# RustAudio/lewton

Hardware: NVIDIA H100
Metric: Msamples/s IMDCT+window+OLA, 2048-pt long blocks (higher is better)
Workload: dtype f32

## Files before the change

### lewton_b200/csrc/host_objects.cuh

```cuda
#pragma once

struct DevBuf {
    void *p = nullptr;
    size_t cap = 0;
};

struct Staging {
    void *h = nullptr;
    size_t cap = 0;
    cudaEvent_t ev = nullptr;
    bool pending = false;
};

struct ArenaSet {
    DevBuf coeffs, dense, pcm, kinds, ys, vqoff, vqrec;
    cudaEvent_t done = nullptr;
};
constexpr int kHostSets = 2;

struct CachedTables {
    DevTables dt;
    std::vector<float> a, b, c, w;
    std::vector<uint32_t> br;
    std::vector<void *> allocs;
};

struct lwb_ctx {
    int device = 0;
    int sm_count = 0;
    cudaStream_t stream = nullptr;
    cudaStream_t copy_in = nullptr, copy_out = nullptr;
    cudaEvent_t ev_in[64] = {}, ev_done[65] = {};
    DevBuf runs_buf[2];
    cudaEvent_t ev_desc[2] = {}, ev_kdone[2] = {};
    int runs_par = 0;
    uint32_t ticket_next = 0;
    uint64_t epoch = 0;
    uint64_t state_gen = 1;
    std::string err;
    uint64_t launches = 0;
    uint64_t kernel_launches[LWB_KERNEL_COUNT] = {};
    std::vector<PcmSpan> pcm_spans;
    std::vector<PcmCopy> pcm_copies;
    std::deque<CachedTables> tables;
    DevBuf spec, segtab, magic, x, desc, chains, ticket, cdesc, cbytes;
    DevBuf floor0;
    ArenaSet host_sets[kHostSets];
    int host_next = 0;
    ArenaSet ordered;
    Staging stage[3];
    int stage_next = 0;
    std::vector<void *> stage_old;
    uint64_t tickets_issued = 0, tickets_done = 0;
    std::deque<cudaEvent_t> ticket_events;
    std::vector<cudaEvent_t> spare_events;
    bool pinned_only = false;
    void *h_desc = nullptr;
    size_t h_desc_cap = 0;
    size_t x_cap_elems = (size_t)64 << 20;
};

struct lwb_setup {
    lwb_ctx *ctx = nullptr;
    DevSetup host;
    DevSetup *d_setup = nullptr;
    std::vector<void *> allocs;
    uint8_t channels = 0, bs0 = 0, bs1 = 0;
    uint32_t n_modes = 0;
    uint32_t n_mappings = 0;
    std::vector<DevMapping> mappings;
    std::vector<uint8_t> floor_types;
    std::vector<DevFloor0> floor0;
    mutable bool streams_opened = false;
    bool floor0_described(uint32_t fi) const { return fi < floor0.size() && floor0[fi].order != 0; }
};

struct RowCopy { const float *src; float *dst; uint32_t n4, pad; };
struct ChainShape { unsigned warps; size_t smem; int n1max, wpc, np; };

struct Step {
    int kernel;
    const void *desc;
    size_t n;
    const float *pack;
};

struct StepArgs {
    void *pcm = nullptr;
    int out_format = LWB_OUT_F32_PLANAR;
    const float *w_short = nullptr;
    int ls = 0;
    int mid_kb = 0;
    ChainShape chain = {};
    const uint8_t *bytes = nullptr;
    bool residue = false;
    const float *coeffs = nullptr, *dense = nullptr;
    const uint8_t *kinds = nullptr;
    const uint32_t *ys = nullptr;
    const float *zero = nullptr;
};
// ... 10 lines not shown
    bool dense = false;
    bool floor0 = false;
};

struct lwb_plan {
    lwb_ctx *ctx = nullptr;
    lwb_chain *chains = nullptr;
    size_t n_chains = 0;
    lwb_batch_io io;
    bool captured = false;
    uint64_t gen = 0;
    FrontStages front;
    DevBuf pro, mix;
    StepArgs args;
    std::vector<Step> steps;
};

struct lwb_stream {
    lwb_ctx *ctx = nullptr;
    const lwb_setup *setup = nullptr;
    float *d_state = nullptr;
    bool has = false;
    uint32_t plen = 0;
    uint64_t busy_epoch = 0;
};

static void capture(lwb_plan *plan, uint64_t gen, const FrontStages &front, const StepArgs &args, std::vector<Step> steps)
{
    plan->captured = true;
    plan->gen = gen;
    plan->front = front;
    for (size_t i = 0; i < plan->n_chains && front.n; i++)
        if (!plan->chains[i].stream->setup->floor0.empty()) plan->front.floor0 = true;
    plan->args = args;
    plan->steps = std::move(steps);
}


static inline void set_stream_state(lwb_stream *s, bool has, uint32_t plen)
{
    if (s->has != has || s->plen != plen) {
        s->has = has;
        s->plen = plen;
        s->ctx->state_gen++;
    }
}

static int fail(lwb_ctx *ctx, int code, const char *what, cudaError_t e = cudaSuccess)
{
    if (ctx) {
        ctx->err = what;
        if (e != cudaSuccess) {
            ctx->err += ": ";
            ctx->err += cudaGetErrorString(e);
        }
    }
    return code;
}

static inline void count_launch(lwb_ctx *ctx, int kernel_id)
{
    ctx->launches++;
    ctx->kernel_launches[kernel_id]++;
}

#define CU(ctx, call)                                                        \
// ... 211 lines not shown
```

### lewton_b200/csrc/kernel_long.cuh

```cuda
#pragma once
#include <stdint.h>

#if defined(__CUDACC__)
#include <cuda_runtime.h>
#define LWB_HD __host__ __device__ __forceinline__
#else
#define LWB_HD inline
#endif

namespace lwb {

constexpr int kLongBs = 11;
constexpr int kLongN = 2048;
constexpr int kLongN2 = 1024;

struct alignas(16) LongRun {
    const float *in;
    void *out;
    float *state;
    uint32_t in_stride;
    uint32_t n_packets;
    uint8_t has_prev;
    uint8_t write_state;
    uint8_t dummy;
    uint8_t first_short;
    uint8_t last_short;
    uint8_t pad[3];
    float *state_out;
};
static_assert(sizeof(LongRun) == 48, "LongRun is copied by TMA in 16-byte units");

struct V { float x, y; };

#if defined(__CUDA_ARCH__)
__device__ __forceinline__ V vadd(V a, V b) { return V{__fadd_rn(a.x, b.x), __fadd_rn(a.y, b.y)}; }
__device__ __forceinline__ V vsub(V a, V b) { return V{__fsub_rn(a.x, b.x), __fsub_rn(a.y, b.y)}; }
__device__ __forceinline__ V vmul(V a, V b) { return V{__fmul_rn(a.x, b.x), __fmul_rn(a.y, b.y)}; }
__device__ __forceinline__ V vadd_p(V a, V b) { return V{__fadd_rn(a.x, b.x), __fadd_rn(a.y, b.y)}; }
__device__ __forceinline__ V vsub_p(V a, V b) { return V{__fsub_rn(a.x, b.x), __fsub_rn(a.y, b.y)}; }
__device__ __forceinline__ V vnsub_p(V a, V b) { return V{__fsub_rn(-a.x, b.x), __fsub_rn(-a.y, b.y)}; }
#else
inline V vadd(V a, V b) { return V{a.x + b.x, a.y + b.y}; }
inline V vsub(V a, V b) { return V{a.x - b.x, a.y - b.y}; }
inline V vmul(V a, V b) { return V{a.x * b.x, a.y * b.y}; }
inline V vadd_p(V a, V b) { return vadd(a, b); }
inline V vsub_p(V a, V b) { return vsub(a, b); }
inline V vnsub_p(V a, V b) { return V{-a.x - b.x, -a.y - b.y}; }
#endif

enum {
// ... 389 lines not shown
    }
};

__device__ __forceinline__ uint32_t laneA(int lane, int half) { return 4u * (uint32_t)swz(elemA(lane, 0, half)); }
__device__ __forceinline__ uint32_t laneB(int lane) { return 4u * (uint32_t)swz(elemB(lane, 0, 0)); }
__device__ __forceinline__ uint32_t laneC(int lane, int half) { return 4u * (uint32_t)swz(elemC(lane, 0, half)); }
#define LWB_KA(j) (4u * (uint32_t)swz(64 * (j)))
#define LWB_KB(j, h) (4u * (uint32_t)swz(((h) << 6) | ((j) << 3)))
#define LWB_KC(j) (4u * (uint32_t)swz(j))

struct RunCur {
    const float *in;
    void *out;
    float *state;
    uint32_t in_stride;
    uint32_t flags;
};
__device__ __forceinline__ RunCur run_cur(const LongRun &r)
{
    return RunCur{r.in, r.out, r.state, r.in_stride,
                  (uint32_t)(r.has_prev ? 1u : 0u) | (r.write_state ? 2u : 0u) | (r.dummy ? 4u : 0u) |
                      (r.first_short ? 8u : 0u) | (r.last_short ? 16u : 0u)};
}
struct RunCurS : RunCur { float *state_out; };
__device__ __forceinline__ RunCurS run_cur_s(const LongRun &r)
{
    RunCurS c;
    static_cast<RunCur &>(c) = run_cur(r);
    c.flags |= r.first_short == 2 ? 32u : 0u;
    c.state_out = r.state_out ? r.state_out : r.state;
    return c;
}

__device__ __forceinline__ int16_t d_sample_i16(float v)
{
    short r;
    asm("cvt.rzi.s16.f32 %0, %1;" : "=h"(r) : "f"(__fmul_rn(v, 32768.0f)));
    return (int16_t)r;
}
__device__ __forceinline__ void st_pcm(float *p, float v) { __stcs(p, v); }
__device__ __forceinline__ void st_pcm(int16_t *p, float v) { __stcs(reinterpret_cast<short *>(p), (short)d_sample_i16(v)); }

template <int NB, bool FIRST, typename OutT, typename RC = RunCur>
__device__ __forceinline__ void out_stage(const TwMix &tw, int lane, const V O[NB][8], const V E[NB][8], V pe[NB][8],
                                          const RC cur[NB], OutT *out[NB], const float *s_state)
{
// ... 142 lines not shown
    uint32_t desc_parity = 0;
    RunCur cur[NB];
    uint32_t npk;

    auto issue_stage = [&](uint32_t stage, const LongRun *r, uint32_t pkt) {
        const uint32_t bar = bars_s + 8 * stage;
        mbar_expect_tx(bar, kLongStageBytes);
#pragma unroll
        for (int b = 0; b < NB; b++)
            tma_load_1d(tiles_s + stage * kLongStageBytes + b * kLongTileBytes,
                        r[b].in + (size_t)pkt * r[b].in_stride, kLongTileBytes, bar);
    };
    auto issue_stage_cur = [&](uint32_t stage, uint32_t pkt) {
        const uint32_t bar = bars_s + 8 * stage;
        mbar_expect_tx(bar, kLongStageBytes);
#pragma unroll
        for (int b = 0; b < NB; b++)
            tma_load_1d(tiles_s + stage * kLongStageBytes + b * kLongTileBytes,
                        cur[b].in + (size_t)pkt * cur[b].in_stride, kLongTileBytes, bar);
    };
    auto issue_state = [&](const float *const st[NB], const uint32_t has[NB]) {
        uint32_t bytes = 0;
#pragma unroll
        for (int b = 0; b < NB; b++) bytes += has[b] ? kLongTileBytes : 0;
        mbar_expect_tx(bar_state, bytes);
#pragma unroll
        for (int b = 0; b < NB; b++)
            if (has[b]) tma_load_1d(state_s + b * kLongTileBytes, st[b], kLongTileBytes, bar_state);
    };

    {
        uint32_t idx = 0;
        if (lane == 0) idx = atomicAdd(ticket, 1u);
        idx = __shfl_sync(0xffffffffu, idx, 0);
        if (idx >= n_groups) return;
#pragma unroll
        for (int b = 0; b < NB; b++) cur[b] = run_cur(runs[idx * NB + b]);
        npk = runs[idx * NB].n_packets;
        if (lane == 0) {
            fence_proxy_async();
            const float *st[NB];
            uint32_t has[NB];
#pragma unroll
            for (int b = 0; b < NB; b++) { st[b] = cur[b].state; has[b] = cur[b].flags & 1u; }
            issue_state(st, has);
            for (; lc < (uint32_t)kLongRing && lc < npk; lc++) issue_stage_cur(lc, lc);
            nx_idx = atomicAdd(ticket, 1u);
        }
    }

    for (;;) {
        V pe[NB][8];
#pragma unroll
        for (int b = 0; b < NB; b++)
#pragma unroll
            for (int j = 0; j < 8; j++) pe[b][j] = V{0.f, 0.f};
        OutT *out[NB];
#pragma unroll
        for (int b = 0; b < NB; b++) out[b] = static_cast<OutT *>(cur[b].out);

        for (uint32_t p = 0; p < npk; p++) {
            const uint32_t stage_s = tiles_s + slot_i * kLongStageBytes;
            mbar_wait(bars_s + 8 * slot_i, (phase_bits >> slot_i) & 1u);
            phase_bits ^= 1u << slot_i;

            V O[NB][8], E[NB][8];
            {
// ... 67 lines not shown
                        lc++;
                    } else {
                        if (nx_stage == 1) {
                            mbar_wait(bar_desc, desc_parity);
                            desc_parity ^= 1u;
                            nx_stage = 2;
                            nx_npk = s_next[0].n_packets;
                            nx_lc = 0;
                        }
                        if (nx_stage == 2 && nx_lc < nx_npk) {
                            fence_proxy_async();
                            issue_stage(tgt, s_next, nx_lc);
                            nx_lc++;
                        }
                    }
                }
            }
            phase_c_fft<NB>(tw, O, E);
            if (p > 0) {
                out_stage<NB, false, OutT>(tw, lane, O, E, pe, cur, out, s_state);
            } else {
                mbar_wait(bar_state, (phase_bits >> 30) & 1u);
                phase_bits ^= 1u << 30;
                if (NB == 1 && (cur[0].flags & 8u))
                    out_first_short<NB, OutT>(tw, lane, O, E, pe, cur, out, s_state, w_short, ls);
                else
                    out_stage<NB, true, OutT>(tw, lane, O, E, pe, cur, out, s_state);
                __syncwarp();
            }
#pragma unroll
            for (int b = 0; b < NB; b++)
                if (p > 0 || (cur[b].flags & 1u)) out[b] += (p == 0 && (cur[b].flags & 8u)) ? kLongN2 - ls : kLongN2;
            if (lane == 0 && nx_stage == 2 && !nx_state_issued) {
                const float *st[NB];
                uint32_t has[NB];
#pragma unroll
                for (int b = 0; b < NB; b++) { st[b] = s_next[b].state; has[b] = s_next[b].has_prev; }
                fence_proxy_async();
                issue_state(st, has);
                nx_state_issued = 1;
            }
            slot_i = (slot_i + 1 == (uint32_t)kLongRing) ? 0 : slot_i + 1;
        }
#pragma unroll
        for (int b = 0; b < NB; b++) {
            if ((cur[b].flags & 16u)) {
                const bool emitted = (npk > 1 || (cur[b].flags & 1u)) && !(cur[b].flags & 4u);
                const bool keep = (cur[b].flags & 6u) == 2u;
#pragma unroll
                for (int j = 0; j < 8; j++) {
                    const int r64 = 64 * rev3(j);
#pragma unroll
                    for (int h = 0; h < 2; h++) {
                        const float v = ((j & 1) != 0) == (h == 0) ? pe[b][j].x : pe[b][j].y;
                        const int m = r64 + (h ? 63 - lane : lane);
                        if (m < ls) {
                            if (emitted) st_pcm(out[b] + m, v);
                        } else if (keep && m < kLongN2 - ls) {
                            cur[b].state[m - ls] = v;
                            cur[b].state[kLongN2 - 1 - ls - m] = v;
                        }
                    }
                }
            } else if ((cur[b].flags & 6u) == 2u) {
                float *s_lo = cur[b].state + lane, *s_hi = cur[b].state + 63 - lane;
#pragma unroll
                for (int j = 0; j < 8; j++) {
                    const int r64 = 64 * rev3(j);
                    const float vx = (j & 1) ? pe[b][j].x : pe[b][j].y, vy = (j & 1) ? pe[b][j].y : pe[b][j].x;
                    s_lo[r64] = vx; s_hi[r64] = vy;
                    s_hi[960 - r64] = vx; s_lo[960 - r64] = vy;
                }
            }
        }
        uint32_t st_ = 0, nlc = 0;
        if (lane == 0) {
            if (nx_stage == 0) {
                if (nx_idx < n_groups) {
                    fence_proxy_async();
                    mbar_expect_tx(bar_desc, NB * (uint32_t)sizeof(LongRun));
                    tma_load_1d(next_s, runs + (size_t)nx_idx * NB, NB * (uint32_t)sizeof(LongRun), bar_desc);
                    nx_stage = 1;
                } else {
                    nx_stage = 3;
                }
            }
            if (nx_stage == 1) {
                mbar_wait(bar_desc, desc_parity);
                desc_parity ^= 1u;
                nx_stage = 2;
                nx_npk = s_next[0].n_packets;
                nx_lc = 0;
            }
            if (nx_stage == 2 && !nx_state_issued) {
                const float *st[NB];
                uint32_t has[NB];
#pragma unroll
                for (int b = 0; b < NB; b++) { st[b] = s_next[b].state; has[b] = s_next[b].has_prev; }
                fence_proxy_async();
                issue_state(st, has);
            }
            st_ = nx_stage;
            nlc = nx_lc;
        }
        st_ = __shfl_sync(0xffffffffu, st_, 0);
        nlc = __shfl_sync(0xffffffffu, nlc, 0);
        if (st_ != 2) break;
        __syncwarp();
#pragma unroll
        for (int b = 0; b < NB; b++) cur[b] = run_cur(s_next[b]);
        npk = s_next[0].n_packets;
        __syncwarp();
        lc = nlc;
        nx_stage = 0; nx_lc = 0; nx_npk = 0; nx_state_issued = 0;
        if (lane == 0) {
            fence_proxy_async();
            for (uint32_t k = lc; k < (uint32_t)kLongRing && k < npk; k++) {
                issue_stage_cur((slot_i + k) % kLongRing, k);
                lc = k + 1;
            }
            nx_idx = atomicAdd(ticket, 1u);
        }
    }
}

constexpr int kLongLs256 = (kLongN - 256) / 4;
constexpr int kLongFetch = 3;
constexpr int kLongDescSlots = kLongFetch + kLongRing + 3;
constexpr int kLongSlopeMax = 512;
constexpr size_t kLongSmemBytesS = 2048 + (size_t)kLongWarps * (kLongRing + 1) * kLongTileBytes + (size_t)kLongPackFloats * 4 +
                                   kLongWarps * (kLongRing + 2) * 8 + (size_t)kLongWarps * kLongDescSlots * sizeof(LongRun) +
                                   kLongSlopeMax * sizeof(float) + 64;

// ... 218 lines not shown
```

### lewton_b200/csrc/lwb_api.cu

```cuda
#include <cuda_runtime.h>
#include <sched.h>
#include <sys/syscall.h>
#include <unistd.h>

#include <algorithm>
#include <cctype>
#include <cstdio>
#include <cstdlib>
#include <cstring>
#include <deque>
#include <new>
#include <string>
#include <vector>

#include "kernel_long.cuh"
#include "kernel_short.cuh"
#include "kernel_mid.cuh"
#include "kernels_generic.cuh"
#include "kernel_chain.cuh"
#include "kernel_prologue.cuh"
#include "kernel_floor0.cuh"
#include "lwb_common.h"
#include "pcm_copy_plan.h"
#include "../../include/lewton_frontend.h"
// ... 55 lines not shown
    short_kernel_configure();
    mid_kernel_configure();
    prologue_kernel_configure();
    *out = ctx;
    return LWB_OK;
}

static cudaError_t sync_all_streams(lwb_ctx *ctx)
{
    cudaError_t e = cudaStreamSynchronize(ctx->stream);
    for (cudaStream_t s : {ctx->copy_in, ctx->copy_out}) {
        const cudaError_t e2 = s ? cudaStreamSynchronize(s) : cudaSuccess;
        if (e == cudaSuccess) e = e2;
    }
    return e;
}

extern "C" void lwb_ctx_destroy(lwb_ctx *ctx)
{
    if (!ctx) return;
    cudaSetDevice(ctx->device);
    sync_all_streams(ctx);
    for (DevBuf *b : {&ctx->spec, &ctx->segtab, &ctx->magic, &ctx->x, &ctx->desc, &ctx->chains, &ctx->ticket, &ctx->runs_buf[0],
                      &ctx->runs_buf[1], &ctx->cdesc, &ctx->cbytes, &ctx->floor0})
        if (b->p) cudaFree(b->p);
    auto free_set = [](ArenaSet &s) {
        for (DevBuf *b : {&s.coeffs, &s.dense, &s.pcm, &s.kinds, &s.ys, &s.vqoff, &s.vqrec})
            if (b->p) cudaFree(b->p);
        if (s.done) cudaEventDestroy(s.done);
    };
    for (ArenaSet &s : ctx->host_sets) free_set(s);
    free_set(ctx->ordered);
    for (cudaEvent_t e : ctx->ticket_events) cudaEventDestroy(e);
    for (cudaEvent_t e : ctx->spare_events) cudaEventDestroy(e);
    for (CachedTables &ct : ctx->tables)
        for (void *p : ct.allocs) cudaFree(p);
    if (ctx->h_desc) cudaFreeHost(ctx->h_desc);
    for (void *h : ctx->stage_old) cudaFreeHost(h);
    for (Staging &st : ctx->stage) {
        if (st.h) cudaFreeHost(st.h);
        if (st.ev) cudaEventDestroy(st.ev);
    }
    for (cudaEvent_t e : ctx->ev_in) if (e) cudaEventDestroy(e);
    for (cudaEvent_t e : ctx->ev_done) if (e) cudaEventDestroy(e);
    for (int k = 0; k < 2; k++) {
        if (ctx->ev_desc[k]) cudaEventDestroy(ctx->ev_desc[k]);
        if (ctx->ev_kdone[k]) cudaEventDestroy(ctx->ev_kdone[k]);
// ... 386 lines not shown
    if (!s) return;
    cudaSetDevice(s->ctx->device);
    sync_all_streams(s->ctx);
    cudaFree(s->d_state);
    delete s;
}

extern "C" int lwb_stream_reset(lwb_stream *s)
{
    if (!s) return LWB_ERR_INVALID;
    set_stream_state(s, false, 0);
    return LWB_OK;
}
extern "C" int lwb_stream_is_empty(const lwb_stream *s) { return (!s || !s->has) ? 1 : 0; }
extern "C" uint32_t lwb_stream_state_len(const lwb_stream *s) { return (s && s->has) ? s->plen : 0; }

extern "C" int lwb_stream_clone(const lwb_stream *s, lwb_stream **out)
{
    if (!s || !out) return LWB_ERR_INVALID;
    int rc = lwb_stream_open(s->ctx, s->setup, out);
    if (rc) return rc;
    (*out)->has = s->has;
    (*out)->plen = s->plen;
    lwb_ctx *ctx = s->ctx;
    CU(ctx, cudaMemcpyAsync((*out)->d_state, s->d_state,
                            s->setup->channels * state_stride(s->setup) * sizeof(float),
                            cudaMemcpyDeviceToDevice, ctx->stream));
    return LWB_OK;
}

extern "C" int lwb_stream_export_state(lwb_stream *s, float *out)
{
    if (!s || !out) return LWB_ERR_INVALID;
    if (!s->has) return LWB_OK;
    lwb_ctx *ctx = s->ctx;
    CU(ctx, cudaSetDevice(ctx->device));
    CU(ctx, cudaMemcpy2DAsync(out, s->plen * sizeof(float), s->d_state, state_stride(s->setup) * sizeof(float),
                              s->plen * sizeof(float), s->setup->channels, cudaMemcpyDeviceToHost, ctx->stream));
    CU(ctx, cudaStreamSynchronize(ctx->stream));
    return LWB_OK;
}

extern "C" int lwb_stream_import_state(lwb_stream *s, const float *data, uint32_t len)
{
    if (!s || (!data && len)) return LWB_ERR_INVALID;
    if (len > state_stride(s->setup)) return LWB_ERR_BUFFER;
    lwb_ctx *ctx = s->ctx;
    CU(ctx, cudaSetDevice(ctx->device));
    if (len) {
        CU(ctx, cudaMemcpy2DAsync(s->d_state, state_stride(s->setup) * sizeof(float), data, len * sizeof(float),
                                  len * sizeof(float), s->setup->channels, cudaMemcpyHostToDevice, ctx->stream));
        CU(ctx, cudaStreamSynchronize(ctx->stream));
    }
    s->ctx->state_gen++;
    s->has = true;
    s->plen = len;
    return LWB_OK;
}

extern "C" int lwb_decoded_sample_count(const lwb_setup *su, uint8_t mode, int prev_flag, int next_flag,
                                        uint32_t *n_samples)
{
    if (!su || !n_samples) return LWB_ERR_INVALID;
    Geom g;
    int rc = geometry(su, mode, prev_flag, next_flag, &g);
    if (rc) return rc;
    *n_samples = g.rs - g.ls;
    return LWB_OK;
}

#include "path_generic.cuh"
#include "path_long.cuh"
#include "path_chain.cuh"
#include "path_mixed.cuh"
#include "path_mid.cuh"

using BatchPath = int (*)(lwb_ctx *, lwb_chain *, size_t, const lwb_batch_io *, bool *, lwb_plan *);
static const BatchPath kBatchPaths[] = {try_long, try_mid, try_mixed, try_chain};
constexpr size_t kNumBatchPaths = sizeof(kBatchPaths) / sizeof(kBatchPaths[0]);

static size_t first_batch_path()
{
    const char *fg = getenv("LWB_FORCE_GENERIC");
    if (!fg) return 0;
    return std::strcmp(fg, "1") == 0 ? kNumBatchPaths : kNumBatchPaths - 1;
}

static int queue_batch(lwb_ctx *ctx, lwb_chain *chains, size_t n_chains, const lwb_batch_io *io, lwb_plan *prepared)
{
    if (!ctx || (!chains && n_chains) || !io) return LWB_ERR_INVALID;
    if (io->entry != LWB_ENTRY_SPECTRUM && io->entry != LWB_ENTRY_RESIDUE && io->entry != LWB_ENTRY_VQ) return fail(ctx, LWB_ERR_INVALID, "bad entry");
    if (io->memory != LWB_MEM_HOST && io->memory != LWB_MEM_DEVICE) return fail(ctx, LWB_ERR_INVALID, "bad memory space");
    if (io->out_format < 0 || io->out_format > LWB_OUT_I16_INTERLEAVED) return fail(ctx, LWB_ERR_INVALID, "bad out_format");
    if (n_chains == 0) return LWB_OK;
    if ((!io->coeffs && io->entry != LWB_ENTRY_VQ) || !io->pcm) return fail(ctx, LWB_ERR_INVALID, "null arena");
    if (io->entry == LWB_ENTRY_VQ && (!io->vq_runs || !io->vq_run_offsets || !io->vq_entries || !io->vq_entry_offsets || !io->floor_kind))
        return fail(ctx, LWB_ERR_INVALID, "VQ entry needs vq_runs, vq_entries, their offsets and floor_kind");
    CU(ctx, cudaSetDevice(ctx->device));
    const uint64_t epoch = ++ctx->epoch;
    const unsigned C = chains[0].stream ? chains[0].stream->setup->channels : 0;
    for (size_t i = 0; i < n_chains; i++) {
        lwb_chain *c = &chains[i];
        if (!c->stream || c->stream->ctx != ctx || (c->n_packets && !c->mode_numbers))
            return fail(ctx, LWB_ERR_INVALID, "chain: bad stream or mode list");
        if (c->stream->busy_epoch == epoch) return fail(ctx, LWB_ERR_INVALID, "a stream appears in two chains of one batch");
        c->stream->busy_epoch = epoch;
        if (io->entry != LWB_ENTRY_SPECTRUM) {
            if (c->stream->setup->channels != C) return fail(ctx, LWB_ERR_INVALID, "residue batches need one channel count");
            if (!io->floor_kind) return fail(ctx, LWB_ERR_INVALID, "residue entry needs floor_kind");
        }
    }
    if (prepared) prepared->captured = false;
    for (size_t k = first_batch_path(); k < kNumBatchPaths; k++) {
        bool handled = false;
        const int rc = kBatchPaths[k](ctx, chains, n_chains, io, &handled, prepared);
        if (rc || handled) return rc;
    }
    std::vector<PlanChain> plan(n_chains);
    std::vector<ChainWalk> walks(n_chains);
    BatchExtent ext;
    int rc;
    for (size_t i = 0; i < n_chains; i++) {
        lwb_chain *c = &chains[i];
        PlanChain &pc = plan[i];
        pc.c = c;
        pc.pk.reserve(c->n_packets);
        walks[i] = walk_chain(c, [&](uint32_t, const Geom &g, bool has, uint32_t plen, uint64_t coeff, uint64_t pos) {
            pc.pk.push_back(PlanPacket{g, has ? plen : 0, coeff, pos});
        });
        set_chain_result(c, walks[i]);
        if ((rc = ext.add(ctx, io, c, walks[i].done, walks[i].coeff_end, walks[i].n_samples))) return rc;
    }
    if ((rc = ext.finish(ctx, io))) return rc;
    if (!ext.empty()) {
        BatchArenas ar;
        if ((rc = ar.open(ctx, io, ext, C, false)) || (rc = ar.upload(0, ext)) || (rc = run_generic(ctx, plan, io, ar, ext.need_floor0)) ||
            (rc = ar.download(0, chains, 0, n_chains, ext)) || (rc = ar.finish()))
            return rc;
    }
    commit_stream_states(chains, walks);
    return LWB_OK;
}

static int decode_chains_impl(lwb_ctx *ctx, lwb_chain *chains, size_t n_chains, const lwb_batch_io *io, lwb_plan *prepared,
// ... 228 lines not shown
```

### lewton_b200/csrc/path_chain.cuh

```cuda
#pragma once

static size_t chain_smem(unsigned maxc, int n1max, int np)
{
    return (size_t)maxc * ((size_t)np * n1max + n1max / 2) * 4 + 8 * (LWB_MAX_POSTS + 1) * 2 * 2 + 64;
}
static int chain_np(unsigned maxc, int n1max, int wpc, bool residue)
{
    if (residue || wpc != 1) return 1;
    int np = 4;
    while (np > 1 && chain_smem(maxc, n1max, np) > 64 * 1024) np >>= 1;
    return np;
}
static ChainShape chain_shape(unsigned maxc, int n1max, bool residue)
{
    int wpc = std::max(1, std::min(8, n1max / 1024));
    while (wpc > 1 && (unsigned)wpc * maxc > 32) wpc >>= 1;
    const int np = chain_np(maxc, n1max, wpc, residue);
    return ChainShape{maxc * wpc, chain_smem(maxc, n1max, np), n1max, wpc, np};
}

__global__ void k_row_copy(const RowCopy *__restrict__ rc)
{
    const RowCopy c = rc[blockIdx.x];
    for (uint32_t i = threadIdx.x; i < c.n4; i += blockDim.x)
        reinterpret_cast<float4 *>(c.dst)[i] = reinterpret_cast<const float4 *>(c.src)[i];
}

static void chain_desc(const lwb_chain *c, uint32_t p0, uint32_t n, bool has, uint32_t plen, uint64_t coeff, uint64_t pos, uint32_t byte_off,
                       ChainDesc *d)
{
    const lwb_stream *s = c->stream;
    const lwb_setup *su = s->setup;
    std::memset(d, 0, sizeof(*d));
    d->setup = su->d_setup;
    d->state = s->d_state;
    d->coeff_off = coeff;
    d->out_off = c->out_offset + pos;
    d->out_stride = c->out_stride;
    d->pkt_index = c->packet_index + p0;
    d->n_packets = n;
    d->byte_off = byte_off;
    d->state_stride = (uint32_t)state_stride(su);
    d->plen0 = (uint16_t)plen;
    d->has0 = has;
    d->channels = (uint8_t)su->channels;
}

static int chain_floor0_curves(lwb_ctx *ctx, const BatchArenas &ar, const BatchExtent &ext, const lwb_chain *chains, size_t n_chains,
// ... 93 lines not shown
```

### lewton_b200/csrc/path_long.cuh

```cuda
#pragma once

struct LongItem {
    const lwb_chain *c;
    uint32_t P;
    bool has_prev;
};

template <typename Run>
static void cut_run(const Run &whole, size_t cuts, size_t first_emit, size_t n2, size_t esz, Run *w)
{
    const size_t P = whole.n_packets;
    for (size_t k = 0; k < cuts; k++) {
        const size_t p0 = P * k / cuts, p1 = P * (k + 1) / cuts;
        Run &r = w[k];
        std::memset(&r, 0, sizeof(r));
        r.in_stride = whole.in_stride;
        r.state = whole.state;
        r.write_state = (k + 1 == cuts);
        if (k == 0) {
            r.in = whole.in;
            r.out = whole.out;
            r.n_packets = (uint32_t)(p1 - p0);
            r.has_prev = whole.has_prev;
        } else {
            const size_t primer = p0 - 1;
            r.in = whole.in + primer * whole.in_stride;
            r.out = (char *)whole.out + (first_emit + primer * n2) * esz;
            r.n_packets = (uint32_t)(p1 - p0 + 1);
            r.has_prev = 0;
        }
    }
}

template <typename Run>
static void channel_run(const lwb_chain *c, unsigned ch, size_t n2, const float *in, char *pcm, size_t esz, uint32_t n, bool has,
                        size_t first_emit, size_t cuts, Run *w)
{
    const lwb_stream *s = c->stream;
    const lwb_setup *su = s->setup;
    const unsigned C = su->channels;
    cut_run(Run{in + (size_t)ch * n2, pcm + (c->out_offset + (size_t)ch * c->out_stride) * esz, s->d_state + (size_t)ch * state_stride(su),
                (uint32_t)(C * n2), n, has},
            cuts, first_emit, n2, esz, w);
}

static void long_runs_of(const LongItem &it, size_t cuts, const float *coeffs, char *pcm, size_t esz, LongRun *&w)
{
    for (unsigned ch = 0; ch < it.c->stream->setup->channels; ch++, w += cuts)
        channel_run(it.c, ch, kLongN2, coeffs + it.c->coeff_offset, pcm, esz, it.P, it.has_prev, it.has_prev ? kLongN2 : 0, cuts, w);
}

static bool batch_is_uniform_long(const lwb_chain *chains, size_t n_chains, const lwb_batch_io *io)
{
    if (!fused_layout(chains, n_chains, io)) return false;
    const float *pack = nullptr;
    for (size_t i = 0; i < n_chains; i++) {
        const lwb_chain *c = &chains[i];
        const lwb_stream *s = c->stream;
        const lwb_setup *su = s->setup;
        if (su->bs1 != kLongBs || !su->host.tab[1].pack) return false;
        if (pack && pack != su->host.tab[1].pack) return false;
        pack = su->host.tab[1].pack;
        if (s->has && s->plen != (uint32_t)kLongN2) return false;
        for (uint32_t k = 0; k < c->n_packets; k++) {
            const uint8_t m = c->mode_numbers[k];
            if (m >= su->n_modes || !su->host.mode_blockflag[m]) return false;
            if (c->prev_window_flags && !c->prev_window_flags[k]) return false;
            if (c->next_window_flags && !c->next_window_flags[k]) return false;
        }
    }
    return true;
}

static int uniform_extent(lwb_ctx *ctx, const lwb_batch_io *io, lwb_chain *chains, size_t i0, size_t i1, uint32_t n2, BatchExtent *ext)
{
    for (size_t i = i0; i < i1; i++) {
        lwb_chain *c = &chains[i];
        c->status = LWB_OK;
        c->packets_done = c->n_packets;
        c->n_samples = c->n_packets ? (c->n_packets - (c->stream->has ? 0u : 1u)) * n2 : 0u;
    }
    int rc = LWB_OK;
    for (size_t i = i0; i < i1 && !rc; i++) {
        const lwb_chain *c = &chains[i];
        rc = ext->add(ctx, io, c, c->n_packets, c->coeff_offset + (uint64_t)c->n_packets * c->stream->setup->channels * n2, c->n_samples);
    }
    return rc;
}

static void commit_uniform_states(lwb_chain *chains, size_t n_chains, uint32_t n2)
{
    for (size_t i = 0; i < n_chains; i++)
        if (chains[i].n_packets) set_stream_state(chains[i].stream, true, n2);
}

struct LongRuns {
    struct Chunk { size_t r0, nr; };
    std::vector<Chunk> chunks;
    Staging *st = nullptr;
    LongRun *h = nullptr, *d = nullptr;
    size_t n = 0;
    int par = 0;
    bool own = false;
};

static int long_build_runs(lwb_ctx *ctx, const lwb_chain *chains, size_t n_chains, size_t n_chunks, const float *coeffs, char *pcm,
                           size_t esz, DevBuf *own, LongRuns *lr)
{
    std::vector<LongItem> items;
    items.reserve(n_chains);
    size_t chan_chains = 0;
    for (size_t i = 0; i < n_chains; i++) {
        const lwb_chain *c = &chains[i];
        items.push_back(LongItem{c, c->n_packets, c->stream->has});
        if (c->n_packets) chan_chains += c->stream->setup->channels;
    }
    const size_t warp_slots = (size_t)ctx->sm_count * kLongWarps * kLongNB;
    size_t target_runs = warp_slots * 4;
    if (const char *e = getenv("LWB_LONG_TARGET_RUNS")) target_runs = (size_t)atol(e);
    const size_t min_run = 8;
    int rc;
    std::vector<size_t> cuts(items.size(), 1);
    size_t total_runs = 0;
    for (size_t i = 0; i < items.size(); i++) {
        if (!items[i].P) { cuts[i] = 0; continue; }
        const size_t per_launch = std::max<size_t>(1, chan_chains / n_chunks);
        size_t k = 1;
        if (per_launch < target_runs) k = (target_runs + per_launch - 1) / per_launch;
        cuts[i] = std::max<size_t>(1, std::min(k, items[i].P / min_run));
        total_runs += cuts[i] * items[i].c->stream->setup->channels;
    }
    const size_t cap_runs = total_runs * (kLongNB > 1 ? 2 : 1) + kLongNB;
    if ((rc = acquire_staging(ctx, cap_runs * sizeof(LongRun), &lr->st))) return rc;
    lr->par = ctx->runs_par;
    ctx->runs_par ^= 1;
    DevBuf &rb = own ? *own : ctx->runs_buf[lr->par];
    lr->own = own != nullptr;
// ... 17 lines not shown
        for (size_t i = i0; i < i1; i++)
            if (items[i].P) long_runs_of(items[i], cuts[i], coeffs, pcm, esz, gen);
        if (kLongNB == 1) {
            w = gen;
        } else {
            bool sorted = true;
            for (size_t i = 1; i < tmp.size() && sorted; i++) sorted = tmp[i].n_packets == tmp[0].n_packets;
            order.resize(tmp.size());
            for (uint32_t i = 0; i < order.size(); i++) order[i] = i;
            if (!sorted)
                std::stable_sort(order.begin(), order.end(),
                                 [&](uint32_t a, uint32_t b) { return tmp[a].n_packets < tmp[b].n_packets; });
            size_t i = 0;
            while (i < order.size()) {
                size_t j = i;
                while (j < order.size() && tmp[order[j]].n_packets == tmp[order[i]].n_packets) j++;
                for (size_t q = i; q < j; q++) *w++ = tmp[order[q]];
                size_t fill = (kLongNB - (j - i) % kLongNB) % kLongNB;
                while (fill--) {
                    LongRun d = tmp[order[j - 1]];
                    d.dummy = 1;
                    d.write_state = 0;
                    d.has_prev = 0;
                    *w++ = d;
                }
                i = j;
            }
        }
        lr->chunks.push_back(LongRuns::Chunk{(size_t)(w0 - h_runs), (size_t)(w - w0)});
    }
    lr->n = (size_t)(w - h_runs);
    return LWB_OK;
}

static int long_upload_runs(lwb_ctx *ctx, const LongRuns &lr, cudaStream_t ds)
{
    int rc;
    if (lr.own && ds != ctx->stream && (rc = order_copies_behind_compute(ctx))) return rc;
    CU(ctx, cudaStreamWaitEvent(ds, ctx->ev_kdone[lr.par], 0));
    if ((rc = upload_staging(ctx, lr.st, lr.h, lr.d, lr.n * sizeof(LongRun), ds))) return rc;
    CU(ctx, cudaEventRecord(ctx->ev_desc[lr.par], ds));
    CU(ctx, cudaStreamWaitEvent(ctx->stream, ctx->ev_desc[lr.par], 0));
    return LWB_OK;
}

static int try_long(lwb_ctx *ctx, lwb_chain *chains, size_t n_chains, const lwb_batch_io *io, bool *handled, lwb_plan *plan)
{
    *handled = false;
    if (!batch_is_uniform_long(chains, n_chains, io)) return LWB_OK;
    *handled = true;
    BatchExtent ext;
    int rc;
    if ((rc = uniform_extent(ctx, io, chains, 0, n_chains, kLongN2, &ext)) || (rc = ext.finish(ctx, io))) return rc;
    if (ext.empty()) return LWB_OK;
    const unsigned C = chains[0].stream->setup->channels;
    const bool residue = io->entry != LWB_ENTRY_SPECTRUM, host = io->memory == LWB_MEM_HOST;
    const float *pack = chains[0].stream->setup->host.tab[1].pack;
    const size_t n_chunks = host ? host_chunks((size_t)(ext.c_hi - ext.c_lo) * 4, n_chains) : 1;
    const bool cap = plan && !host;
    BatchArenas ar;
    if ((rc = ar.open(ctx, io, ext, C, true))) return rc;
    const float *in = ar.coeffs;
    FrontStages fs;
    if (residue) {
        size_t n_pk = 0;
        for (size_t i = 0; i < n_chains; i++) n_pk += chains[i].n_packets;
        if ((rc = ensure(ctx, ctx->spec, (size_t)(ext.c_hi - ext.c_lo) * 4))) return rc;
        fs = front_stages_of(ext, C, kLongN, n_pk);
        if (plan && plan->pro.p && plan->front.pk == plan->pro.p && plan->front.n == n_pk) {
            fs.pk = plan->front.pk;
            fs.fast = plan->front.fast;
        } else if ((rc = stage_front_packets(ctx, ar, chains, n_chains, plan ? plan->pro : ctx->desc, 0, &fs))) {
            return rc;
        }
        if (plan) plan->front = fs;
        in = (const float *)ctx->spec.p - ext.c_lo;
    }
    StepArgs args;
    args.pcm = ar.pcm;
    args.out_format = io->out_format;
    std::vector<Step> steps;
    LongRuns lr;
    uint64_t gen = 0;
    size_t pk0 = 0;
    for (size_t k = 0; k < n_chunks; k++) {
        const size_t i0 = n_chains * k / n_chunks, i1 = n_chains * (k + 1) / n_chunks;
        BatchExtent ke;
        ke.scan = false;
        if ((rc = uniform_extent(ctx, io, chains, i0, i1, kLongN2, &ke))) return rc;
        if (ke.empty()) continue;
        size_t npk = 0;
        for (size_t i = i0; i < i1; i++) npk += chains[i].n_packets;
        if ((rc = ar.upload(k, ke)) || (residue && (rc = front_stages_launch(ctx, ar, fs, pk0, npk)))) return rc;
        if (!lr.d) {
            if ((rc = long_build_runs(ctx, chains, n_chains, n_chunks, in, ar.pcm, elem_size(io->out_format), cap ? &plan->mix : nullptr, &lr)) ||
                (rc = long_upload_runs(ctx, lr, host ? ctx->copy_in : ctx->copy_out)))
                return rc;
            gen = ctx->state_gen;
        }
        steps.assign(1, Step{LWB_KERNEL_LONG, lr.d + lr.chunks[k].r0, lr.chunks[k].nr / kLongNB, pack});
        if ((rc = run_steps(ctx, args, steps)) || (rc = ar.download(k, chains, i0, i1, ke))) return rc;
        pk0 += npk;
    }
    CU(ctx, cudaEventRecord(ctx->ev_kdone[lr.par], ctx->stream));
    if (cap) capture(plan, gen, fs, args, std::move(steps));
    if ((rc = ar.finish())) return rc;
    commit_uniform_states(chains, n_chains, kLongN2);
    return LWB_OK;
}
```

### lewton_b200/csrc/path_mid.cuh

```cuda
#pragma once

struct MidGroup { LongRun r[4]; uint32_t n_packets; };

static int try_mid(lwb_ctx *ctx, lwb_chain *chains, size_t n_chains, const lwb_batch_io *io, bool *handled, lwb_plan *plan)
{
    *handled = false;
    const uint64_t gen_at_entry = ctx->state_gen;
    if (getenv("LWB_NO_MID")) return LWB_OK;
    const bool vq = io->entry == LWB_ENTRY_VQ, residue = io->entry != LWB_ENTRY_SPECTRUM;
    if (vq) return LWB_OK;
    if (!fused_layout(chains, n_chains, io)) return LWB_OK;
    const size_t esz = elem_size(io->out_format);
    const float *pack = nullptr;
    int kb = 0;
    size_t n_runs = 0;
    for (size_t i = 0; i < n_chains; i++) {
        const lwb_chain *c = &chains[i];
        const lwb_setup *su = c->stream->setup;
        if (su->channels > 8 || (su->bs1 != 10 && su->bs1 != 9) || !su->host.tab[1].pack) return LWB_OK;
        if (pack && pack != su->host.tab[1].pack) return LWB_OK;
        pack = su->host.tab[1].pack;
        kb = 11 - su->bs1;
        const uint32_t n_blk = 2048u >> kb, n2_blk = n_blk >> 1;
        if (c->stream->has && c->stream->plen != n2_blk) return LWB_OK;
// ... 63 lines not shown
            g.r[k].write_state = 0;
            g.r[k].has_prev = 0;
        }
        groups.push_back(g);
    }
    const size_t Wg = (size_t)static_deal_grid(groups.size(), kLongWarps, ctx->sm_count) * kLongWarps;
    balance_static_deal(groups.data(), groups.size(), Wg, tmp_g);
    const size_t bytes = groups.size() * NBg * sizeof(LongRun);
    Staging *st;
    if ((rc = acquire_staging(ctx, bytes, &st))) return rc;
    LongRun *h = (LongRun *)st->h;
    for (size_t k = 0; k < groups.size(); k++)
        for (size_t b = 0; b < NBg; b++) h[NBg * k + b] = groups[k].r[b];
    if (bytes > off_pro) return fail(ctx, LWB_ERR_INVALID, "internal: more run groups than runs");
    if ((rc = upload_staging(ctx, st, h, dbuf.p, bytes, ctx->stream))) return rc;
    StepArgs args;
    args.pcm = ar.pcm;
    args.out_format = io->out_format;
    args.mid_kb = kb;
    std::vector<Step> steps(1, Step{LWB_KERNEL_MID, dbuf.p, groups.size(), pack});
    if ((rc = run_steps(ctx, args, steps))) return rc;
    if (cap) capture(plan, gen_at_entry, fs, args, std::move(steps));
    if ((rc = ar.download(0, chains, 0, n_chains, ext)) || (rc = ar.finish())) return rc;
    commit_uniform_states(chains, n_chains, (uint32_t)kMidN2);
    return LWB_OK;
}
```

Baseline: 317,100.

## Store only half of symmetric long-block overlap state and mirror on load

When the long path runs from a captured plan, it writes only half of each channel's 1024-float overlap state. This relies on the state being mirror-symmetric after a long block. On the next long run, only that half is loaded by TMA and then mirrored in shared memory. Other paths, and the host state getter, first expand the half state back to a full row with a mirroring row-copy kernel. The aim is to cut the per-run state write and read traffic, at the cost of extra shared-memory shuffling, proxy fences, and more state-tracking complexity.

```diff
diff --git a/lewton_b200/csrc/host_objects.cuh b/lewton_b200/csrc/host_objects.cuh
--- a/lewton_b200/csrc/host_objects.cuh
+++ b/lewton_b200/csrc/host_objects.cuh
@@ -44,6 +44,7 @@
     std::vector<PcmCopy> pcm_copies;
     std::deque<CachedTables> tables;
     DevBuf spec, segtab, magic, x, desc, chains, ticket, cdesc, cbytes;
+    DevBuf mirror;
     DevBuf floor0;
     ArenaSet host_sets[kHostSets];
     int host_next = 0;
@@ -75,7 +76,7 @@
     bool floor0_described(uint32_t fi) const { return fi < floor0.size() && floor0[fi].order != 0; }
 };
 
-struct RowCopy { const float *src; float *dst; uint32_t n4, pad; };
+struct RowCopy { const float *src; float *dst; uint32_t n4, mirror; };
 struct ChainShape { unsigned warps; size_t smem; int n1max, wpc, np; };
 
 struct Step {
@@ -132,6 +133,8 @@
     float *d_state = nullptr;
     bool has = false;
     uint32_t plen = 0;
+    bool symmetric = false;
+    bool half = false;
     uint64_t busy_epoch = 0;
 };
 
@@ -147,11 +150,13 @@
 }
 
 
-static inline void set_stream_state(lwb_stream *s, bool has, uint32_t plen)
-{
-    if (s->has != has || s->plen != plen) {
+static inline void set_stream_state(lwb_stream *s, bool has, uint32_t plen, bool symmetric = false, bool half = false)
+{
+    if (s->has != has || s->plen != plen || s->symmetric != symmetric || s->half != half) {
         s->has = has;
         s->plen = plen;
+        s->symmetric = symmetric;
+        s->half = half;
         s->ctx->state_gen++;
     }
 }
diff --git a/lewton_b200/csrc/kernel_long.cuh b/lewton_b200/csrc/kernel_long.cuh
--- a/lewton_b200/csrc/kernel_long.cuh
+++ b/lewton_b200/csrc/kernel_long.cuh
@@ -25,7 +25,9 @@
     uint8_t dummy;
     uint8_t first_short;
     uint8_t last_short;
-    uint8_t pad[3];
+    uint8_t half_in;
+    uint8_t half_out;
+    uint8_t pad;
     float *state_out;
 };
 static_assert(sizeof(LongRun) == 48, "LongRun is copied by TMA in 16-byte units");
@@ -461,6 +463,12 @@
                   (uint32_t)(r.has_prev ? 1u : 0u) | (r.write_state ? 2u : 0u) | (r.dummy ? 4u : 0u) |
                       (r.first_short ? 8u : 0u) | (r.last_short ? 16u : 0u)};
 }
+__device__ __forceinline__ RunCur run_cur_l(const LongRun &r)
+{
+    RunCur c = run_cur(r);
+    c.flags |= (r.half_in ? 64u : 0u) | (r.half_out ? 128u : 0u);
+    return c;
+}
 struct RunCurS : RunCur { float *state_out; };
 __device__ __forceinline__ RunCurS run_cur_s(const LongRun &r)
 {
@@ -649,12 +657,13 @@
     auto issue_state = [&](const float *const st[NB], const uint32_t has[NB]) {
         uint32_t bytes = 0;
 #pragma unroll
-        for (int b = 0; b < NB; b++) bytes += has[b] ? kLongTileBytes : 0;
+        for (int b = 0; b < NB; b++) bytes += has[b];
         mbar_expect_tx(bar_state, bytes);
 #pragma unroll
         for (int b = 0; b < NB; b++)
-            if (has[b]) tma_load_1d(state_s + b * kLongTileBytes, st[b], kLongTileBytes, bar_state);
+            if (has[b]) tma_load_1d(state_s + b * kLongTileBytes, st[b], has[b], bar_state);
     };
+    auto state_bytes = [](bool has, bool half) -> uint32_t { return has ? (half ? kLongTileBytes / 2 : kLongTileBytes) : 0u; };
 
     {
         uint32_t idx = 0;
@@ -662,14 +671,14 @@
         idx = __shfl_sync(0xffffffffu, idx, 0);
         if (idx >= n_groups) return;
 #pragma unroll
-        for (int b = 0; b < NB; b++) cur[b] = run_cur(runs[idx * NB + b]);
+        for (int b = 0; b < NB; b++) cur[b] = run_cur_l(runs[idx * NB + b]);
         npk = runs[idx * NB].n_packets;
         if (lane == 0) {
             fence_proxy_async();
             const float *st[NB];
             uint32_t has[NB];
 #pragma unroll
-            for (int b = 0; b < NB; b++) { st[b] = cur[b].state; has[b] = cur[b].flags & 1u; }
+            for (int b = 0; b < NB; b++) { st[b] = cur[b].state; has[b] = state_bytes(cur[b].flags & 1u, cur[b].flags & 64u); }
             issue_state(st, has);
             for (; lc < (uint32_t)kLongRing && lc < npk; lc++) issue_stage_cur(lc, lc);
             nx_idx = atomicAdd(ticket, 1u);
@@ -783,6 +792,19 @@
             } else {
                 mbar_wait(bar_state, (phase_bits >> 30) & 1u);
                 phase_bits ^= 1u << 30;
+#pragma unroll
+                for (int b = 0; b < NB; b++) {
+                    if ((cur[b].flags & 65u) == 65u) {
+                        float4 *row = reinterpret_cast<float4 *>(s_state + b * kLongN2);
+#pragma unroll 1
+                        for (int k = 0; k < kLongN2 / 8 / 32; k++) {
+                            const float4 v = row[lane + 32 * k];
+                            row[kLongN2 / 4 - 1 - lane - 32 * k] = make_float4(v.w, v.z, v.y, v.x);
+                        }
+                        fence_proxy_async();
+                    }
+                }
+                __syncwarp();
                 if (NB == 1 && (cur[0].flags & 8u))
                     out_first_short<NB, OutT>(tw, lane, O, E, pe, cur, out, s_state, w_short, ls);
                 else
@@ -796,7 +818,7 @@
                 const float *st[NB];
                 uint32_t has[NB];
 #pragma unroll
-                for (int b = 0; b < NB; b++) { st[b] = s_next[b].state; has[b] = s_next[b].has_prev; }
+                for (int b = 0; b < NB; b++) { st[b] = s_next[b].state; has[b] = state_bytes(s_next[b].has_prev, s_next[b].half_in); }
                 fence_proxy_async();
                 issue_state(st, has);
                 nx_state_issued = 1;
@@ -830,7 +852,9 @@
                     const int r64 = 64 * rev3(j);
                     const float vx = (j & 1) ? pe[b][j].x : pe[b][j].y, vy = (j & 1) ? pe[b][j].y : pe[b][j].x;
                     s_lo[r64] = vx; s_hi[r64] = vy;
-                    s_hi[960 - r64] = vx; s_lo[960 - r64] = vy;
+                    if (!(cur[b].flags & 128u)) {
+                        s_hi[960 - r64] = vx; s_lo[960 - r64] = vy;
+                    }
                 }
             }
         }
@@ -857,7 +881,7 @@
                 const float *st[NB];
                 uint32_t has[NB];
 #pragma unroll
-                for (int b = 0; b < NB; b++) { st[b] = s_next[b].state; has[b] = s_next[b].has_prev; }
+                for (int b = 0; b < NB; b++) { st[b] = s_next[b].state; has[b] = state_bytes(s_next[b].has_prev, s_next[b].half_in); }
                 fence_proxy_async();
                 issue_state(st, has);
             }
@@ -869,7 +893,7 @@
         if (st_ != 2) break;
         __syncwarp();
 #pragma unroll
-        for (int b = 0; b < NB; b++) cur[b] = run_cur(s_next[b]);
+        for (int b = 0; b < NB; b++) cur[b] = run_cur_l(s_next[b]);
         npk = s_next[0].n_packets;
         __syncwarp();
         lc = nlc;
diff --git a/lewton_b200/csrc/lwb_api.cu b/lewton_b200/csrc/lwb_api.cu
--- a/lewton_b200/csrc/lwb_api.cu
+++ b/lewton_b200/csrc/lwb_api.cu
@@ -101,7 +101,7 @@
     cudaSetDevice(ctx->device);
     sync_all_streams(ctx);
     for (DevBuf *b : {&ctx->spec, &ctx->segtab, &ctx->magic, &ctx->x, &ctx->desc, &ctx->chains, &ctx->ticket, &ctx->runs_buf[0],
-                      &ctx->runs_buf[1], &ctx->cdesc, &ctx->cbytes, &ctx->floor0})
+                      &ctx->runs_buf[1], &ctx->cdesc, &ctx->cbytes, &ctx->floor0, &ctx->mirror})
         if (b->p) cudaFree(b->p);
     auto free_set = [](ArenaSet &s) {
         for (DevBuf *b : {&s.coeffs, &s.dense, &s.pcm, &s.kinds, &s.ys, &s.vqoff, &s.vqrec})
@@ -534,6 +534,8 @@
     if (rc) return rc;
     (*out)->has = s->has;
     (*out)->plen = s->plen;
+    (*out)->symmetric = s->symmetric;
+    (*out)->half = s->half;
     lwb_ctx *ctx = s->ctx;
     CU(ctx, cudaMemcpyAsync((*out)->d_state, s->d_state,
                             s->setup->channels * state_stride(s->setup) * sizeof(float),
@@ -547,9 +549,15 @@
     if (!s->has) return LWB_OK;
     lwb_ctx *ctx = s->ctx;
     CU(ctx, cudaSetDevice(ctx->device));
+    const size_t w = s->half ? s->plen / 2 : s->plen;
     CU(ctx, cudaMemcpy2DAsync(out, s->plen * sizeof(float), s->d_state, state_stride(s->setup) * sizeof(float),
-                              s->plen * sizeof(float), s->setup->channels, cudaMemcpyDeviceToHost, ctx->stream));
+                              w * sizeof(float), s->setup->channels, cudaMemcpyDeviceToHost, ctx->stream));
     CU(ctx, cudaStreamSynchronize(ctx->stream));
+    if (s->half)
+        for (unsigned ch = 0; ch < s->setup->channels; ch++) {
+            float *row = out + (size_t)ch * s->plen;
+            for (size_t m = 0; m < w; m++) row[s->plen - 1 - m] = row[m];
+        }
     return LWB_OK;
 }
 
@@ -567,6 +575,8 @@
     s->ctx->state_gen++;
     s->has = true;
     s->plen = len;
+    s->symmetric = false;
+    s->half = false;
     return LWB_OK;
 }
 
@@ -586,6 +596,29 @@
 #include "path_chain.cuh"
 #include "path_mixed.cuh"
 #include "path_mid.cuh"
+
+static int expand_half_states(lwb_ctx *ctx, const lwb_chain *chains, size_t n_chains)
+{
+    size_t n = 0;
+    for (size_t i = 0; i < n_chains; i++)
+        if (chains[i].stream->half) n += chains[i].stream->setup->channels;
+    if (!n) return LWB_OK;
+    Staging *st;
+    int rc;
+    if ((rc = ensure(ctx, ctx->mirror, n * sizeof(RowCopy))) || (rc = acquire_staging(ctx, n * sizeof(RowCopy), &st))) return rc;
+    RowCopy *h = (RowCopy *)st->h;
+    for (size_t i = 0; i < n_chains; i++) {
+        lwb_stream *s = chains[i].stream;
+        if (!s->half) continue;
+        for (unsigned ch = 0; ch < s->setup->channels; ch++) {
+            float *row = s->d_state + (size_t)ch * state_stride(s->setup);
+            *h++ = RowCopy{row, row, s->plen / 8, 1};
+        }
+        set_stream_state(s, s->has, s->plen, s->symmetric, false);
+    }
+    if ((rc = upload_staging(ctx, st, st->h, ctx->mirror.p, n * sizeof(RowCopy), ctx->stream))) return rc;
+    return launch(ctx, LWB_KERNEL_ROW_COPY, k_row_copy, dim3((unsigned)n), dim3(64), 0, (const RowCopy *)ctx->mirror.p);
+}
 
 using BatchPath = int (*)(lwb_ctx *, lwb_chain *, size_t, const lwb_batch_io *, bool *, lwb_plan *);
 static const BatchPath kBatchPaths[] = {try_long, try_mid, try_mixed, try_chain};
@@ -623,15 +656,21 @@
         }
     }
     if (prepared) prepared->captured = false;
+    int rc;
+    bool whole = false;
     for (size_t k = first_batch_path(); k < kNumBatchPaths; k++) {
+        if (kBatchPaths[k] != try_long && !whole) {
+            if ((rc = expand_half_states(ctx, chains, n_chains))) return rc;
+            whole = true;
+        }
         bool handled = false;
-        const int rc = kBatchPaths[k](ctx, chains, n_chains, io, &handled, prepared);
+        rc = kBatchPaths[k](ctx, chains, n_chains, io, &handled, prepared);
         if (rc || handled) return rc;
     }
+    if (!whole && (rc = expand_half_states(ctx, chains, n_chains))) return rc;
     std::vector<PlanChain> plan(n_chains);
     std::vector<ChainWalk> walks(n_chains);
     BatchExtent ext;
-    int rc;
     for (size_t i = 0; i < n_chains; i++) {
         lwb_chain *c = &chains[i];
         PlanChain &pc = plan[i];
diff --git a/lewton_b200/csrc/path_chain.cuh b/lewton_b200/csrc/path_chain.cuh
--- a/lewton_b200/csrc/path_chain.cuh
+++ b/lewton_b200/csrc/path_chain.cuh
@@ -22,8 +22,13 @@
 __global__ void k_row_copy(const RowCopy *__restrict__ rc)
 {
     const RowCopy c = rc[blockIdx.x];
-    for (uint32_t i = threadIdx.x; i < c.n4; i += blockDim.x)
-        reinterpret_cast<float4 *>(c.dst)[i] = reinterpret_cast<const float4 *>(c.src)[i];
+    const float4 *src = reinterpret_cast<const float4 *>(c.src);
+    float4 *dst = reinterpret_cast<float4 *>(c.dst);
+    for (uint32_t i = threadIdx.x; i < c.n4; i += blockDim.x) {
+        const float4 v = src[i];
+        if (c.mirror) dst[2 * c.n4 - 1 - i] = make_float4(v.w, v.z, v.y, v.x);
+        else dst[i] = v;
+    }
 }
 
 static void chain_desc(const lwb_chain *c, uint32_t p0, uint32_t n, bool has, uint32_t plen, uint64_t coeff, uint64_t pos, uint32_t byte_off,
diff --git a/lewton_b200/csrc/path_long.cuh b/lewton_b200/csrc/path_long.cuh
--- a/lewton_b200/csrc/path_long.cuh
+++ b/lewton_b200/csrc/path_long.cuh
@@ -4,6 +4,8 @@
     const lwb_chain *c;
     uint32_t P;
     bool has_prev;
+    bool symmetric;
+    bool half_out;
 };
 
 template <typename Run>
@@ -46,8 +48,11 @@
 
 static void long_runs_of(const LongItem &it, size_t cuts, const float *coeffs, char *pcm, size_t esz, LongRun *&w)
 {
-    for (unsigned ch = 0; ch < it.c->stream->setup->channels; ch++, w += cuts)
+    for (unsigned ch = 0; ch < it.c->stream->setup->channels; ch++, w += cuts) {
         channel_run(it.c, ch, kLongN2, coeffs + it.c->coeff_offset, pcm, esz, it.P, it.has_prev, it.has_prev ? kLongN2 : 0, cuts, w);
+        w[0].half_in = it.has_prev && it.symmetric;
+        w[cuts - 1].half_out = it.half_out;
+    }
 }
 
 static bool batch_is_uniform_long(const lwb_chain *chains, size_t n_chains, const lwb_batch_io *io)
@@ -88,10 +93,10 @@
     return rc;
 }
 
-static void commit_uniform_states(lwb_chain *chains, size_t n_chains, uint32_t n2)
+static void commit_uniform_states(lwb_chain *chains, size_t n_chains, uint32_t n2, bool symmetric, bool half)
 {
     for (size_t i = 0; i < n_chains; i++)
-        if (chains[i].n_packets) set_stream_state(chains[i].stream, true, n2);
+        if (chains[i].n_packets) set_stream_state(chains[i].stream, true, n2, symmetric, half);
 }
 
 struct LongRuns {
@@ -105,14 +110,14 @@
 };
 
 static int long_build_runs(lwb_ctx *ctx, const lwb_chain *chains, size_t n_chains, size_t n_chunks, const float *coeffs, char *pcm,
-                           size_t esz, DevBuf *own, LongRuns *lr)
+                           size_t esz, DevBuf *own, bool half_out, LongRuns *lr)
 {
     std::vector<LongItem> items;
     items.reserve(n_chains);
     size_t chan_chains = 0;
     for (size_t i = 0; i < n_chains; i++) {
         const lwb_chain *c = &chains[i];
-        items.push_back(LongItem{c, c->n_packets, c->stream->has});
+        items.push_back(LongItem{c, c->n_packets, c->stream->has, c->stream->symmetric, half_out});
         if (c->n_packets) chan_chains += c->stream->setup->channels;
     }
     const size_t warp_slots = (size_t)ctx->sm_count * kLongWarps * kLongNB;
@@ -176,6 +181,7 @@
                     d.dummy = 1;
                     d.write_state = 0;
                     d.has_prev = 0;
+                    d.half_in = d.half_out = 0;
                     *w++ = d;
                 }
                 i = j;
@@ -212,6 +218,7 @@
     const float *pack = chains[0].stream->setup->host.tab[1].pack;
     const size_t n_chunks = host ? host_chunks((size_t)(ext.c_hi - ext.c_lo) * 4, n_chains) : 1;
     const bool cap = plan && !host;
+    const bool half_out = plan != nullptr;
     BatchArenas ar;
     if ((rc = ar.open(ctx, io, ext, C, true))) return rc;
     const float *in = ar.coeffs;
@@ -247,7 +254,7 @@
         for (size_t i = i0; i < i1; i++) npk += chains[i].n_packets;
         if ((rc = ar.upload(k, ke)) || (residue && (rc = front_stages_launch(ctx, ar, fs, pk0, npk)))) return rc;
         if (!lr.d) {
-            if ((rc = long_build_runs(ctx, chains, n_chains, n_chunks, in, ar.pcm, elem_size(io->out_format), cap ? &plan->mix : nullptr, &lr)) ||
+            if ((rc = long_build_runs(ctx, chains, n_chains, n_chunks, in, ar.pcm, elem_size(io->out_format), cap ? &plan->mix : nullptr, half_out, &lr)) ||
                 (rc = long_upload_runs(ctx, lr, host ? ctx->copy_in : ctx->copy_out)))
                 return rc;
             gen = ctx->state_gen;
@@ -259,6 +266,6 @@
     CU(ctx, cudaEventRecord(ctx->ev_kdone[lr.par], ctx->stream));
     if (cap) capture(plan, gen, fs, args, std::move(steps));
     if ((rc = ar.finish())) return rc;
-    commit_uniform_states(chains, n_chains, kLongN2);
+    commit_uniform_states(chains, n_chains, kLongN2, true, half_out);
     return LWB_OK;
 }
diff --git a/lewton_b200/csrc/path_mid.cuh b/lewton_b200/csrc/path_mid.cuh
--- a/lewton_b200/csrc/path_mid.cuh
+++ b/lewton_b200/csrc/path_mid.cuh
@@ -109,6 +109,6 @@
     if ((rc = run_steps(ctx, args, steps))) return rc;
     if (cap) capture(plan, gen_at_entry, fs, args, std::move(steps));
     if ((rc = ar.download(0, chains, 0, n_chains, ext)) || (rc = ar.finish())) return rc;
-    commit_uniform_states(chains, n_chains, (uint32_t)kMidN2);
+    commit_uniform_states(chains, n_chains, (uint32_t)kMidN2, false, false);
     return LWB_OK;
 }
diff --git a/profiles/state_traffic_probe.py b/profiles/state_traffic_probe.py
--- /dev/null
+++ b/profiles/state_traffic_probe.py
@@ -0,0 +1,96 @@
+#!/usr/bin/env python3
+import argparse
+import json
+import os
+import subprocess
+import sys
+
+import numpy as np
+
+ROOT = os.path.dirname(os.path.dirname(os.path.abspath(__file__)))
+sys.path.insert(0, ROOT)
+
+N2, C, STREAMS = 1024, 2, 4096
+
+
+def card():
+    q = subprocess.run(["nvidia-smi", "--query-gpu=name,power.limit,clocks.max.sm", "--format=csv,noheader", "-i", "0"],
+                       capture_output=True, text=True)
+    return q.stdout.strip() if q.returncode == 0 else f"nvidia-smi failed: {q.stderr.strip()}"
+
+
+def time_shape(L, cabi, torch, ctx, su, stream, P, seconds):
+    gen = torch.Generator(device="cuda").manual_seed(1234)
+    spec = torch.randn((STREAMS, P, C, N2), generator=gen, device="cuda", dtype=torch.float32) * 1e-2
+    stride = P * N2
+    pcm = torch.empty((STREAMS, C, stride), device="cuda", dtype=torch.float32)
+    pwrs = [L.PreviousWindowRight(su) for _ in range(STREAMS)]
+    modes = np.ones(P, np.uint8)
+    chains = [L.ChainSpec(pwrs[s], modes, coeff_offset=s * P * C * N2, out_offset=s * C * stride, out_stride=stride)
+              for s in range(STREAMS)]
+    batch = L.Batch(ctx, chains, cabi.ENTRY_SPECTRUM, cabi.MEM_DEVICE, spec.data_ptr(), pcm.data_ptr(), cabi.OUT_F32_PLANAR)
+    for _ in range(5):
+        batch.run()
+    ctx.synchronize()
+    e0, e1 = torch.cuda.Event(enable_timing=True), torch.cuda.Event(enable_timing=True)
+    e0.record(stream)
+    for _ in range(10):
+        batch.run()
+    e1.record(stream)
+    ctx.synchronize()
+    n = max(20, int(seconds * 1e3 / (e0.elapsed_time(e1) / 10)) + 1)
+    l0 = ctx.launch_count
+    e0.record(stream)
+    for i in range(n):
+        batch.run()
+        if (i & 255) == 255:
+            ctx.synchronize()
+    e1.record(stream)
+    ctx.synchronize()
+    ms = e0.elapsed_time(e1) / n
+    launches = (ctx.launch_count - l0) / n
+    batch.close()
+    for p in pwrs:
+        p.close()
+    del spec, pcm
+    torch.cuda.empty_cache()
+    return ms, n, launches
+
+
+def main():
+    ap = argparse.ArgumentParser()
+    ap.add_argument("--packets", default="8,16,32,64")
+    ap.add_argument("--seconds", type=float, default=1.0)
+    args = ap.parse_args()
+    import torch
+
+    import lewton_b200 as L
+    from lewton_b200 import _cabi as cabi
+
+    gpu = card()
+    ctx = L.Context(0)
+    su = L.Setup(ctx, C, 8, 11, [L.FloorTypeOne(1, [0, 128])], [L.Mapping(C)], [L.ModeInfo(False), L.ModeInfo(True)])
+    stream = torch.cuda.ExternalStream(ctx.cuda_stream, device=torch.device("cuda", 0))
+    sms = torch.cuda.get_device_properties(0).multi_processor_count
+    W = sms * 8
+    Ps = [int(p) for p in args.packets.split(",")]
+    rows = []
+    for P in Ps:
+        ms, n, launches = time_shape(L, cabi, torch, ctx, su, stream, P, args.seconds)
+        rows.append({"P": P, "ms_per_step": ms, "steps": n, "launches_per_step": launches,
+                     "msamples_per_s": STREAMS * P * C * N2 / (ms * 1e-3) / 1e6})
+    x = np.array([r["P"] for r in rows], float)
+    y = np.array([r["ms_per_step"] for r in rows], float) * 1e3
+    slope, icpt = np.polyfit(x, y, 1)
+    resid = y - (slope * x + icpt)
+    runs_per_warp = C * STREAMS / W
+    t_packet, t_run = slope / runs_per_warp, icpt / runs_per_warp
+    print(json.dumps({"gpu": gpu, "sms": sms, "warps": W, "runs_per_warp": runs_per_warp, "shapes": rows,
+                      "t_packet_us": t_packet, "t_run_us": t_run, "t_run_over_t_packet": t_run / t_packet,
+                      "fit_residual_us": [float(r) for r in resid],
+                      "model": "t_step = 8192 / W * (P * t_packet + t_run), least squares over P"}))
+    ctx.close()
+
+
+if __name__ == "__main__":
+    main()
```

After: 324,900 (median of 6 runs). +2.5%, better.
